# damaggu/StableKeypoints

Hardware: AMD Instinct MI355X
Metric: images/sec (token-opt step, 512², N=500 tokens) (higher is better)
Workload: dtype f32

## Files before the change

stablekeypoints_amd/csrc/skp_softmax.hip:

```cpp
#include "skp_common.h"

using namespace skp;

namespace {

template <int TPR, int EPT, bool VEC>
__global__ __launch_bounds__(TPR) void softmax_bwd_kernel(const float* __restrict__ P, float* __restrict__ G,
                                                          long long rows, int cols, float alpha) {
  __shared__ float sred[TPR / WAVE];
  const long long row = blockIdx.x;
  if (row >= rows) return;
  const float* p = P + row * cols;
  float* g = G + row * cols;
  static_assert(!VEC || EPT % 4 == 0, "float4 path needs EPT % 4 == 0");
  float pv[EPT], gv[EPT];
  float dot = 0.0f;
  if (VEC) {
#pragma unroll
    for (int q = 0; q < EPT / 4; ++q) {
      const int e = 4 * (threadIdx.x + q * TPR);
      float4 a = make_float4(0.f, 0.f, 0.f, 0.f), b = a;
      if (e < cols) {
        a = *reinterpret_cast<const float4*>(p + e);
        b = *reinterpret_cast<const float4*>(g + e);
      }
      pv[4 * q] = a.x; pv[4 * q + 1] = a.y; pv[4 * q + 2] = a.z; pv[4 * q + 3] = a.w;
      gv[4 * q] = b.x; gv[4 * q + 1] = b.y; gv[4 * q + 2] = b.z; gv[4 * q + 3] = b.w;
    }
  } else {
#pragma unroll
    for (int q = 0; q < EPT; ++q) {
      const int e = threadIdx.x + q * TPR;
      pv[q] = e < cols ? p[e] : 0.0f;
      gv[q] = e < cols ? g[e] : 0.0f;
    }
  }
#pragma unroll
  for (int q = 0; q < EPT; ++q) dot += pv[q] * gv[q];
  dot = wave_sum(dot);
  if (TPR > WAVE) {
    const int lane = threadIdx.x & (WAVE - 1), wid = threadIdx.x / WAVE;
    if (lane == 0) sred[wid] = dot;
    __syncthreads();
    float t = 0.0f;
#pragma unroll
    for (int w = 0; w < TPR / WAVE; ++w) t += sred[w];
    dot = t;
  }
  if (VEC) {
#pragma unroll
    for (int q = 0; q < EPT / 4; ++q) {
      const int e = 4 * (threadIdx.x + q * TPR);
      if (e < cols)
        *reinterpret_cast<float4*>(g + e) =
            make_float4(alpha * (pv[4 * q] * (gv[4 * q] - dot)), alpha * (pv[4 * q + 1] * (gv[4 * q + 1] - dot)),
                        alpha * (pv[4 * q + 2] * (gv[4 * q + 2] - dot)),
                        alpha * (pv[4 * q + 3] * (gv[4 * q + 3] - dot)));
    }
  } else {
#pragma unroll
    for (int q = 0; q < EPT; ++q) {
      const int e = threadIdx.x + q * TPR;
      if (e < cols) g[e] = alpha * (pv[q] * (gv[q] - dot));
    }
  }
}

template <int TPR, int EPT>
__global__ __launch_bounds__(TPR) void softmax_fwd_kernel(float* __restrict__ S, long long rows, int cols) {
  __shared__ float sred[2][TPR / WAVE];
  const long long row = blockIdx.x;
  if (row >= rows) return;
  float* p = S + row * cols;
  float v[EPT];
  float m = -INFINITY;
#pragma unroll
  for (int q = 0; q < EPT / 4; ++q) {
    const int e = 4 * (threadIdx.x + q * TPR);
    float4 a = make_float4(-INFINITY, -INFINITY, -INFINITY, -INFINITY);
    if (e < cols) a = *reinterpret_cast<const float4*>(p + e);
    v[4 * q] = a.x;
    v[4 * q + 1] = a.y;
    v[4 * q + 2] = a.z;
// ... 92 lines not shown
                                                          const float* __restrict__ V, const float* __restrict__ D,
                                                          float* out, int S, int L, float alpha) {
  constexpr int d = 4 * KS, dp = d + 1;
  __shared__ float sO[64 * dp], sV[64 * dp];
  const int b = blockIdx.z;
  const int r0 = blockIdx.y * 64, k0 = blockIdx.x * 64;
  const int t = threadIdx.x, lane = t & 63, w = t >> 6;
  {
    const float4* gO = reinterpret_cast<const float4*>(dO + ((size_t)b * S + r0) * d);
    const float4* gV = reinterpret_cast<const float4*>(V + ((size_t)b * L + k0) * d);
    for (int e = t; e < 64 * KS; e += 256) {
      const int row = e / KS, c = 4 * (e - row * KS);
      const float4 o = gO[e], v = gV[e];
      float* po = sO + row * dp + c;
      float* pv = sV + row * dp + c;
      po[0] = o.x; po[1] = o.y; po[2] = o.z; po[3] = o.w;
      pv[0] = v.x; pv[1] = v.y; pv[2] = v.z; pv[3] = v.w;
    }
  }
  __syncthreads();
  const float* va = sV + (16 * w + (lane & 15)) * dp + (lane >> 4);
  const float* ob = sO + (lane & 15) * dp + (lane >> 4);
  f32x4a acc[4];
#pragma unroll
  for (int bj = 0; bj < 4; ++bj) acc[bj] = f32x4a{0.f, 0.f, 0.f, 0.f};
#pragma unroll
  for (int ks = 0; ks < KS; ++ks) {
    const float a = va[4 * ks];
#pragma unroll
    for (int bj = 0; bj < 4; ++bj)
      acc[bj] = __builtin_amdgcn_mfma_f32_16x16x4f32(a, ob[16 * bj * dp + 4 * ks], acc[bj], 0, 0, 0);
  }
  const int key = k0 + 16 * w + 4 * (lane >> 4);
#pragma unroll
  for (int bj = 0; bj < 4; ++bj) {
    const int row = r0 + 16 * bj + (lane & 15);
    const float dr = D[(size_t)b * S + row];
    const size_t o = ((size_t)b * S + row) * L + key;
    const float4 p = *reinterpret_cast<const float4*>(P + o);
    *reinterpret_cast<float4*>(out + o) =
        make_float4(alpha * (p.x * (acc[bj][0] - dr)), alpha * (p.y * (acc[bj][1] - dr)),
                    alpha * (p.z * (acc[bj][2] - dr)), alpha * (p.w * (acc[bj][3] - dr)));
  }
}
}

extern "C" int skp_attn_dscore(const float* P, const float* dO, const float* V, const float* D, float* out, int BH,
                               int S, int L, int d, float alpha, void* stream) {
  SKP_CHECK_ARG(P && dO && V && D && out, "null pointer");
  SKP_CHECK_ARG(BH > 0 && S > 0 && L > 0 && d > 0, "non-positive shape");
  SKP_CHECK_ARG(S % 64 == 0 && L % 64 == 0, "S and L must be multiples of 64");
  SKP_CHECK_ARG(((reinterpret_cast<uintptr_t>(P) | reinterpret_cast<uintptr_t>(dO) | reinterpret_cast<uintptr_t>(V) |
                  reinterpret_cast<uintptr_t>(out)) & 15) == 0,
                "tensors must be 16-byte aligned");
  SKP_CHECK_ARG(BH <= 65535 && S / 64 <= 65535, "grid too large");
  const dim3 grid((unsigned)(L / 64), (unsigned)(S / 64), (unsigned)BH);
  hipStream_t st = as_stream(stream);
#define SKP_DS(K) hipLaunchKernelGGL((attn_dscore_kernel<K>), grid, dim3(256), 0, st, P, dO, V, D, out, S, L, alpha)
  switch (d) {
    case 40: SKP_DS(10); break;
    case 64: SKP_DS(16); break;
    case 80: SKP_DS(20); break;
    case 160: SKP_DS(40); break;
    default: SKP_CHECK_ARG(false, "head dim must be 40, 64, 80 or 160");
  }
#undef SKP_DS
  SKP_LAUNCH_CHECK();
  return SKP_OK;
}

struct AttnLay {
  long long sb;
  int rs;
  template <typename T>
  __device__ __forceinline__ T* at(T* base, int bh, int H, int d) const {
    const int b = bh / H;
    return base + (size_t)b * sb + (size_t)(bh - b * H) * d;
  }
};

namespace {

template <int KS, int DB>
__global__ __launch_bounds__(256) void attn_fwd_kernel(const float* __restrict__ Q, const float* __restrict__ K,
                                                       const float* __restrict__ V, float* __restrict__ O,
                                                       float2* __restrict__ ST, int S, int L, float scale, int H,
                                                       AttnLay lq, AttnLay lk, AttnLay lv, AttnLay lo) {
  constexpr int d = 4 * KS, dp = d + 1;
  __shared__ float sK[64 * dp], sV[64 * 16 * DB];
  const int b = blockIdx.y;
  const int r0 = blockIdx.x * 64;
  const int t = threadIdx.x, lane = t & 63, w = t >> 6;
  const int row = r0 + 16 * w + (lane & 15);
  const float* Qb = lq.at(Q, b, H, d);
  const float* Kb = lk.at(K, b, H, d);
  const float* Vb = lv.at(V, b, H, d);
  float qv[KS];
  {
    const float* q = Qb + (size_t)row * lq.rs + (lane >> 4);
#pragma unroll
    for (int ks = 0; ks < KS; ++ks) qv[ks] = q[4 * ks] * scale;
  }
  f32x4a o[DB];
#pragma unroll
  for (int db = 0; db < DB; ++db) o[db] = f32x4a{0.f, 0.f, 0.f, 0.f};
  float m = -INFINITY, l = 0.0f;
  for (int k0 = 0; k0 < L; k0 += 64) {
    __syncthreads();
    {
      for (int e = t; e < 64 * KS; e += 256) {
        const int key = e / KS, c = 4 * (e - key * KS);
        float4 kk = make_float4(0.f, 0.f, 0.f, 0.f), vv = kk;
        if (k0 + key < L) {
          kk = *reinterpret_cast<const float4*>(Kb + (size_t)(k0 + key) * lk.rs + c);
          vv = *reinterpret_cast<const float4*>(Vb + (size_t)(k0 + key) * lv.rs + c);
        }
        float* pk = sK + key * dp + c;
        pk[0] = kk.x; pk[1] = kk.y; pk[2] = kk.z; pk[3] = kk.w;
        *reinterpret_cast<float4*>(sV + key * 16 * DB + c) = vv;
      }
      if constexpr (16 * DB > d)
        for (int e = t; e < 64 * (16 * DB - d); e += 256) {
          const int key = e / (16 * DB - d), c = d + (e - key * (16 * DB - d));
          sV[key * 16 * DB + c] = 0.0f;
        }
    }
    __syncthreads();
    f32x4a s4[4];
#pragma unroll
    for (int c = 0; c < 4; ++c) {
      s4[c] = f32x4a{0.f, 0.f, 0.f, 0.f};
      const float* kr = sK + (16 * c + (lane & 15)) * dp + (lane >> 4);
#pragma unroll
      for (int ks = 0; ks < KS; ++ks) s4[c] = __builtin_amdgcn_mfma_f32_16x16x4f32(kr[4 * ks], qv[ks], s4[c], 0, 0, 0);
    }
    if (k0 + 64 > L) {
#pragma unroll
      for (int c = 0; c < 4; ++c)
#pragma unroll
        for (int r = 0; r < 4; ++r)
          if (k0 + 16 * c + 4 * (lane >> 4) + r >= L) s4[c][r] = -INFINITY;
    }
    float bm = -INFINITY;
#pragma unroll
    for (int c = 0; c < 4; ++c) bm = fmaxf(bm, fmaxf(fmaxf(s4[c][0], s4[c][1]), fmaxf(s4[c][2], s4[c][3])));
    bm = fmaxf(bm, __shfl_xor(bm, 16, 64));
    bm = fmaxf(bm, __shfl_xor(bm, 32, 64));
    const float mn = fmaxf(m, bm);
    const float corr = __expf(m - mn);
    float bs = 0.0f;
#pragma unroll
    for (int c = 0; c < 4; ++c)
#pragma unroll
      for (int r = 0; r < 4; ++r) {
        s4[c][r] = __expf(s4[c][r] - mn);
        bs += s4[c][r];
      }
    bs += __shfl_xor(bs, 16, 64);
    bs += __shfl_xor(bs, 32, 64);
    l = l * corr + bs;
    m = mn;
#pragma unroll
    for (int db = 0; db < DB; ++db) o[db] *= corr;
#pragma unroll
    for (int c = 0; c < 4; ++c)
#pragma unroll
      for (int r = 0; r < 4; ++r) {
        const float* vr = sV + (16 * c + 4 * (lane >> 4) + r) * 16 * DB + (lane & 15);
#pragma unroll
        for (int db = 0; db < DB; ++db)
          o[db] = __builtin_amdgcn_mfma_f32_16x16x4f32(vr[16 * db], s4[c][r], o[db], 0, 0, 0);
      }
  }
  const float inv = 1.0f / l;
  float* orow = lo.at(O, b, H, d) + (size_t)row * lo.rs;
#pragma unroll
  for (int db = 0; db < DB; ++db) {
    const int dd = 16 * db + 4 * (lane >> 4);
    if (dd < d) *reinterpret_cast<float4*>(orow + dd) = make_float4(o[db][0] * inv, o[db][1] * inv, o[db][2] * inv, o[db][3] * inv);
  }
  if (ST != nullptr && lane < 16) ST[(size_t)b * S + row] = make_float2(m, inv);
}

}

namespace {
int attn_fwd_launch(const float* Q, AttnLay lq, const float* K, AttnLay lk, const float* V, AttnLay lv, float* O,
                    AttnLay lo, float* stats, int BH, int H, int S, int L, int d, float scale, void* stream) {
  SKP_CHECK_ARG(Q && K && V && O, "null pointer");
  SKP_CHECK_ARG(BH > 0 && H > 0 && BH % H == 0 && S > 0 && L > 0, "non-positive shape");
  SKP_CHECK_ARG(S % 64 == 0, "S must be a multiple of 64");
  SKP_CHECK_ARG(BH <= 65535, "grid too large");
  SKP_CHECK_ARG(((reinterpret_cast<uintptr_t>(K) | reinterpret_cast<uintptr_t>(V) | reinterpret_cast<uintptr_t>(O)) &
                 15) == 0,
                "tensors must be 16-byte aligned");
  SKP_CHECK_ARG(((lk.rs | lv.rs | lo.rs | lk.sb | lv.sb | lo.sb) & 3) == 0, "K, V, O strides must be multiples of 4");
  SKP_CHECK_ARG((reinterpret_cast<uintptr_t>(stats) & 7) == 0, "stats must be 8-byte aligned");
  const dim3 grid((unsigned)(S / 64), (unsigned)BH);
  hipStream_t st = as_stream(stream);
  float2* ST = reinterpret_cast<float2*>(stats);
#define SKP_AF(KS_, DB_)                                                                                        \
  hipLaunchKernelGGL((attn_fwd_kernel<KS_, DB_>), grid, dim3(256), 0, st, Q, K, V, O, ST, S, L, scale, H, lq, lk, lv, \
                     lo)
  switch (d) {
    case 40: SKP_AF(10, 3); break;
    case 64: SKP_AF(16, 4); break;
    case 80: SKP_AF(20, 5); break;
    default: SKP_CHECK_ARG(false, "head dim must be 40, 64 or 80");
  }
#undef SKP_AF
  SKP_LAUNCH_CHECK();
  return SKP_OK;
}
AttnLay contig(int rows, int d) { return AttnLay{(long long)rows * d, d}; }
}

extern "C" int skp_attn_fwd(const float* Q, const float* K, const float* V, float* O, float* stats, int BH, int S,
                            int L, int d, float scale, void* stream) {
  return attn_fwd_launch(Q, contig(S, d), K, contig(L, d), V, contig(L, d), O, contig(S, d), stats, BH, 1, S, L, d,
                         scale, stream);
}

extern "C" int skp_attn_fwd_bshd(const float* Q, long long q_sb, int q_rs, const float* K, long long k_sb, int k_rs,
                                 const float* V, long long v_sb, int v_rs, float* O, long long o_sb, int o_rs,
                                 float* stats, int B, int H, int S, int L, int d, float scale, void* stream) {
  SKP_CHECK_ARG(B > 0 && H > 0 && (long long)B * H <= 65535, "bad B, H");
  return attn_fwd_launch(Q, AttnLay{q_sb, q_rs}, K, AttnLay{k_sb, k_rs}, V, AttnLay{v_sb, v_rs}, O, AttnLay{o_sb, o_rs},
                         stats, B * H, H, S, L, d, scale, stream);
}

namespace {

template <int KS, int DB, int WPE, bool RC>
__global__ __launch_bounds__(256) __attribute__((amdgpu_waves_per_eu(WPE, WPE))) void attn_bwd_kv_kernel(
    const float* __restrict__ P, const float* __restrict__ dO, const float* __restrict__ Q, const float* __restrict__ V,
    const float* __restrict__ D, float* __restrict__ dS, float* __restrict__ dV, float* __restrict__ dK, int S, int L,
    float alpha, const float* __restrict__ Kt, const float2* __restrict__ ST, float scale, int H, AttnLay lo, AttnLay lq,
    AttnLay lk, AttnLay lv, AttnLay ldv, AttnLay ldk) {
  constexpr int d = 4 * KS, dp = d + 1, dq = 16 * DB + 1;
  __shared__ float sV[64 * dp];
  __shared__ float sK[RC ? 64 * dp : 1];
  __shared__ float2 sST[2][RC ? 64 : 1];
  __shared__ float sO[2][64 * dq], sQ[2][64 * dq];
  __shared__ float sD[2][64];
  const int b = blockIdx.y, k0 = blockIdx.x * 64;
  const int t = threadIdx.x, lane = t & 63, w = t >> 6;
  const float* Vb = lv.at(V, b, H, d);
  const float* dOb = lo.at(dO, b, H, d);
  const float* Qb = lq.at(Q, b, H, d);
  {
    for (int e = t; e < 64 * KS; e += 256) {
      const int key = e / KS, c = 4 * (e - key * KS);
      const bool in = k0 + key < L;
      const float4 v = in ? *reinterpret_cast<const float4*>(Vb + (size_t)(k0 + key) * lv.rs + c)
                          : make_float4(0.f, 0.f, 0.f, 0.f);
      float* p = sV + key * dp + c;
      p[0] = v.x; p[1] = v.y; p[2] = v.z; p[3] = v.w;
      if constexpr (RC) {
        const float4 kk = in ? *reinterpret_cast<const float4*>(lk.at(Kt, b, H, d) + (size_t)(k0 + key) * lk.rs + c)
                             : make_float4(0.f, 0.f, 0.f, 0.f);
        float* pk = sK + key * dp + c;
        pk[0] = kk.x; pk[1] = kk.y; pk[2] = kk.z; pk[3] = kk.w;
      }
    }
    for (int e = t; e < 64 * (dq - d); e += 256) {
      const int row = e / (dq - d), c = d + (e - row * (dq - d));
      sO[0][row * dq + c] = 0.0f; sO[1][row * dq + c] = 0.0f;
      sQ[0][row * dq + c] = 0.0f; sQ[1][row * dq + c] = 0.0f;
    }
  }
  constexpr int NPF = (64 * KS + 255) / 256;
  float4 fo[NPF], fq[NPF];
  float fd = 0.0f;
  float2 fst = make_float2(0.0f, 0.0f);
  const int rl = 16 * w + 4 * (lane >> 4);
  auto fetch = [&](int r0) {
#pragma unroll
    for (int j = 0; j < NPF; ++j) {
      const int e = t + 256 * j;
      if (e < 64 * KS) {
        const int row = e / KS, c = 4 * (e - row * KS);
        fo[j] = *reinterpret_cast<const float4*>(dOb + (size_t)(r0 + row) * lo.rs + c);
        fq[j] = *reinterpret_cast<const float4*>(Qb + (size_t)(r0 + row) * lq.rs + c);
      }
    }
    if (t < 64) {
      fd = D[(size_t)b * S + r0 + t];
      if constexpr (RC) fst = ST[(size_t)b * S + r0 + t];
    }
  };
  auto stash = [&](int buf) {
#pragma unroll
    for (int j = 0; j < NPF; ++j) {
      const int e = t + 256 * j;
      if (e < 64 * KS) {
        const int row = e / KS, c = 4 * (e - row * KS);
        float* po = sO[buf] + row * dq + c;
        float* pq = sQ[buf] + row * dq + c;
        po[0] = fo[j].x; po[1] = fo[j].y; po[2] = fo[j].z; po[3] = fo[j].w;
        pq[0] = fq[j].x; pq[1] = fq[j].y; pq[2] = fq[j].z; pq[3] = fq[j].w;
      }
    }
    if (t < 64) {
      sD[buf][t] = fd;
      if constexpr (RC) sST[buf][t] = fst;
    }
  };
  const float* Pl = P + ((size_t)b * S + rl) * L + k0 + (lane & 15);
  float* dSl = dS + ((size_t)b * S + rl) * L + k0 + (lane & 15);
  f32x4a pc[4];
  if constexpr (!RC) {
#pragma unroll
    for (int bj = 0; bj < 4; ++bj)
#pragma unroll
      for (int r = 0; r < 4; ++r) pc[bj][r] = Pl[(size_t)r * L + 16 * bj];
  }
  fetch(0);
  stash(0);
  f32x4a dv[DB][4], dk[DB][4];
#pragma unroll
  for (int db = 0; db < DB; ++db)
#pragma unroll
    for (int bj = 0; bj < 4; ++bj) {
      dv[db][bj] = f32x4a{0.f, 0.f, 0.f, 0.f};
      dk[db][bj] = f32x4a{0.f, 0.f, 0.f, 0.f};
    }
  for (int r0 = 0, buf = 0; r0 < S; r0 += 64, buf ^= 1) {
    __syncthreads();
    const bool more = r0 + 64 < S;
    f32x4a pn[4];
    if (more) {
      fetch(r0 + 64);
      if constexpr (!RC) {
        const float* Pn = Pl + (size_t)(r0 + 64) * L;
#pragma unroll
        for (int bj = 0; bj < 4; ++bj)
#pragma unroll
          for (int r = 0; r < 4; ++r) pn[bj][r] = Pn[(size_t)r * L + 16 * bj];
      }
    }
    const float* tO = sO[buf];
    const float* tQ = sQ[buf];
    f32x4a dp4[4];
    {
      const float* oa = tO + (16 * w + (lane & 15)) * dq + (lane >> 4);
      const float* vb = sV + (lane & 15) * dp + (lane >> 4);
#pragma unroll
      for (int bj = 0; bj < 4; ++bj) dp4[bj] = f32x4a{0.f, 0.f, 0.f, 0.f};
#pragma unroll
      for (int ks = 0; ks < KS; ++ks) {
        const float a = oa[4 * ks];
#pragma unroll
        for (int bj = 0; bj < 4; ++bj)
          dp4[bj] = __builtin_amdgcn_mfma_f32_16x16x4f32(a, vb[16 * bj * dp + 4 * ks], dp4[bj], 0, 0, 0);
      }
    }
    if constexpr (RC) {
      f32x4a sc[4];
      const float* qa = tQ + (16 * w + (lane & 15)) * dq + (lane >> 4);
      const float* kb = sK + (lane & 15) * dp + (lane >> 4);
#pragma unroll
      for (int bj = 0; bj < 4; ++bj) sc[bj] = f32x4a{0.f, 0.f, 0.f, 0.f};
#pragma unroll
      for (int ks = 0; ks < KS; ++ks) {
        const float a = qa[4 * ks];
#pragma unroll
        for (int bj = 0; bj < 4; ++bj)
          sc[bj] = __builtin_amdgcn_mfma_f32_16x16x4f32(a, kb[16 * bj * dp + 4 * ks], sc[bj], 0, 0, 0);
      }
#pragma unroll
      for (int r = 0; r < 4; ++r) {
        const float2 st = sST[buf][rl + r];
#pragma unroll
        for (int bj = 0; bj < 4; ++bj)
          pc[bj][r] = k0 + 16 * bj + (lane & 15) < L ? __expf(sc[bj][r] * scale - st.x) * st.y : 0.0f;
      }
    }
    f32x4a s4[4];
    float* dSr = dSl + (size_t)r0 * L;
#pragma unroll
    for (int r = 0; r < 4; ++r) {
      const float Dr = sD[buf][rl + r];
#pragma unroll
      for (int bj = 0; bj < 4; ++bj) {
        const float sv = alpha * (pc[bj][r] * (dp4[bj][r] - Dr));
        if (!RC || k0 + 16 * bj + (lane & 15) < L) dSr[(size_t)r * L + 16 * bj] = sv;
        s4[bj][r] = sv;
      }
    }
#pragma unroll
    for (int r = 0; r < 4; ++r) {
      const float* orow = tO + (rl + r) * dq + (lane & 15);
      const float* qrow = tQ + (rl + r) * dq + (lane & 15);
#pragma unroll
      for (int db = 0; db < DB; ++db) {
        const float ao = orow[16 * db], aq = qrow[16 * db];
#pragma unroll
        for (int bj = 0; bj < 4; ++bj) {
          dv[db][bj] = __builtin_amdgcn_mfma_f32_16x16x4f32(ao, pc[bj][r], dv[db][bj], 0, 0, 0);
          dk[db][bj] = __builtin_amdgcn_mfma_f32_16x16x4f32(aq, s4[bj][r], dk[db][bj], 0, 0, 0);
        }
      }
    }
    if (more) {
      stash(buf ^ 1);
      if constexpr (!RC) {
#pragma unroll
        for (int bj = 0; bj < 4; ++bj) pc[bj] = pn[bj];
      }
    }
  }
  __syncthreads();
  float* red = sO[0];
  for (int m = 0; m < 2; ++m) {
#pragma unroll
    for (int db = 0; db < DB; ++db)
#pragma unroll
      for (int bj = 0; bj < 4; ++bj) {
        const f32x4a val = m == 0 ? dv[db][bj] : dk[db][bj];
        *reinterpret_cast<float4*>(red + (w * 64 + lane) * 4) = make_float4(val[0], val[1], val[2], val[3]);
        __syncthreads();
        if (w == 0) {
          float4 acc = *reinterpret_cast<const float4*>(red + lane * 4);
#pragma unroll
          for (int ww = 1; ww < 4; ++ww) {
            const float4 x = *reinterpret_cast<const float4*>(red + (ww * 64 + lane) * 4);
            acc.x += x.x; acc.y += x.y; acc.z += x.z; acc.w += x.w;
          }
          const int dd = 16 * db + 4 * (lane >> 4);
          const int key = k0 + 16 * bj + (lane & 15);
          if (dd < d && key < L) {
            float* dst = m == 0 ? ldv.at(dV, b, H, d) + (size_t)key * ldv.rs : ldk.at(dK, b, H, d) + (size_t)key * ldk.rs;
            *reinterpret_cast<float4*>(dst + dd) = acc;
          }
        }
        __syncthreads();
      }
  }
}

}

extern "C" int skp_attn_bwd_kv(const float* P, const float* dO, const float* Q, const float* V, const float* D,
                               float* dS, float* dV, float* dK, int BH, int S, int L, int d, float alpha,
                               void* stream) {
  SKP_CHECK_ARG(P && dO && Q && V && D && dS && dV && dK, "null pointer");
  SKP_CHECK_ARG(BH > 0 && S > 0 && L > 0, "non-positive shape");
  SKP_CHECK_ARG(S % 64 == 0 && L % 64 == 0, "S and L must be multiples of 64");
  SKP_CHECK_ARG(BH <= 65535, "grid too large");
  SKP_CHECK_ARG(((reinterpret_cast<uintptr_t>(dO) | reinterpret_cast<uintptr_t>(Q) | reinterpret_cast<uintptr_t>(V) |
                  reinterpret_cast<uintptr_t>(dV) | reinterpret_cast<uintptr_t>(dK)) & 15) == 0,
                "tensors must be 16-byte aligned");
  const dim3 grid((unsigned)(L / 64), (unsigned)BH);
  hipStream_t st = as_stream(stream);
  const AttnLay ls = contig(S, d), ll = contig(L, d);
  switch (d) {
#define SKP_BKV(KS_, DB_, W_) \
  hipLaunchKernelGGL((attn_bwd_kv_kernel<KS_, DB_, W_, false>), grid, dim3(256), 0, st, P, dO, Q, V, D, dS, dV, dK, S, L, \
                     alpha, nullptr, nullptr, 0.0f, 1, ls, ls, ll, ll, ll, ll)
    case 40: SKP_BKV(10, 3, 2); break;
    case 64: SKP_BKV(16, 4, 1); break;
    case 80: SKP_BKV(20, 5, 1); break;
#undef SKP_BKV
    default: SKP_CHECK_ARG(false, "head dim must be 40, 64 or 80");
  }
  SKP_LAUNCH_CHECK();
  return SKP_OK;
}

namespace {
int attn_bwd_flash_launch(const float* Q, AttnLay lq, const float* K, AttnLay lk, const float* V, AttnLay lv,
                          const float* dO, AttnLay lo, const float* stats, const float* D, float* dS, float* dV,
                          AttnLay ldv, float* dK, AttnLay ldk, int BH, int H, int S, int L, int d, float scale,
                          void* stream) {
  SKP_CHECK_ARG(Q && K && V && dO && stats && D && dS && dV && dK, "null pointer");
  SKP_CHECK_ARG(BH > 0 && H > 0 && BH % H == 0 && S > 0 && L > 0, "non-positive shape");
  SKP_CHECK_ARG(S % 64 == 0, "S must be a multiple of 64");
  SKP_CHECK_ARG(BH <= 65535, "grid too large");
  SKP_CHECK_ARG(((reinterpret_cast<uintptr_t>(dO) | reinterpret_cast<uintptr_t>(Q) | reinterpret_cast<uintptr_t>(K) |
                  reinterpret_cast<uintptr_t>(V) | reinterpret_cast<uintptr_t>(dV) | reinterpret_cast<uintptr_t>(dK)) &
                 15) == 0 && (reinterpret_cast<uintptr_t>(stats) & 7) == 0,
                "tensors must be 16-byte aligned (stats 8-byte)");
  SKP_CHECK_ARG(((lq.rs | lk.rs | lv.rs | lo.rs | ldv.rs | ldk.rs | lq.sb | lk.sb | lv.sb | lo.sb | ldv.sb | ldk.sb) & 3) == 0,
                "strides must be multiples of 4");
  const dim3 grid((unsigned)((L + 63) / 64), (unsigned)BH);
  hipStream_t st = as_stream(stream);
  const float2* ST = reinterpret_cast<const float2*>(stats);
  switch (d) {
#define SKP_BFL(KS_, DB_, W_) \
  hipLaunchKernelGGL((attn_bwd_kv_kernel<KS_, DB_, W_, true>), grid, dim3(256), 0, st, nullptr, dO, Q, V, D, dS, dV, dK, \
                     S, L, scale, K, ST, scale, H, lo, lq, lk, lv, ldv, ldk)
    case 40: SKP_BFL(10, 3, 2); break;
    case 64: SKP_BFL(16, 4, 1); break;
    case 80: SKP_BFL(20, 5, 1); break;
#undef SKP_BFL
    default: SKP_CHECK_ARG(false, "head dim must be 40, 64 or 80");
  }
  SKP_LAUNCH_CHECK();
  return SKP_OK;
}
}

extern "C" int skp_attn_bwd_flash(const float* Q, const float* K, const float* V, const float* dO, const float* stats,
                                  const float* D, float* dS, float* dV, float* dK, int BH, int S, int L, int d, float scale,
                                  void* stream) {
  const AttnLay ls = contig(S, d), ll = contig(L, d);
  return attn_bwd_flash_launch(Q, ls, K, ll, V, ll, dO, ls, stats, D, dS, dV, ll, dK, ll, BH, 1, S, L, d, scale, stream);
}

extern "C" int skp_attn_bwd_flash_bshd(const float* Q, long long q_sb, int q_rs, const float* K, long long k_sb,
                                       int k_rs, const float* V, long long v_sb, int v_rs, const float* dO,
                                       long long o_sb, int o_rs, const float* stats, const float* D, float* dS,
                                       float* dV, long long dv_sb, int dv_rs, float* dK, long long dk_sb, int dk_rs,
                                       int B, int H, int S, int L, int d, float scale, void* stream) {
  SKP_CHECK_ARG(B > 0 && H > 0 && (long long)B * H <= 65535, "bad B, H");
  return attn_bwd_flash_launch(Q, AttnLay{q_sb, q_rs}, K, AttnLay{k_sb, k_rs}, V, AttnLay{v_sb, v_rs}, dO,
                               AttnLay{o_sb, o_rs}, stats, D, dS, dV, AttnLay{dv_sb, dv_rs}, dK, AttnLay{dk_sb, dk_rs},
                               B * H, H, S, L, d, scale, stream);
}
```

stablekeypoints_amd/ops.py:

```python
import ctypes
import os

import torch

from . import _lib
from ._lib import call, ptr, stream

F32 = torch.float32

_TIMER = None


def set_kernel_timer(timer):
    global _TIMER
    _TIMER = timer


class _NoTimer:
    def __enter__(self):
        return self

    def __exit__(self, *a):
        return False

# ... 1042 lines not shown
        dy = _c(dy)
        dres = None if dpass is None else _c16(dpass)
        C = x.shape[-1]
        dx = torch.empty_like(x)
        call("skp_layernorm_bwd_add", ptr(x), ptr(dy), ptr(w), ptr(stats), x.numel() // C, C, ptr(dres), ptr(dx),
             stream(x.device))
        return dx, None, None, None


def layer_norm_res(x, weight, bias, eps):
    _lib.require_device(x)
    C = x.shape[-1]
    if (x.dtype != F32 or C % 4 or C > 2048 or weight is None or bias is None or weight.requires_grad
            or bias.requires_grad or x.numel() == 0 or x.numel() // C < LN_MIN_ROWS):
        return torch.nn.functional.layer_norm(x, (C,), weight, bias, eps), x
    return LayerNormRes.apply(x, weight, bias, float(eps))


LN_MIN_ROWS = 2048


def layer_norm(x, weight, bias, eps):
    _lib.require_device(x)
    C = x.shape[-1]
    if (x.dtype != F32 or C % 4 or C > 2048 or weight is None or bias is None or weight.requires_grad
            or bias.requires_grad or x.numel() == 0 or x.numel() // C < LN_MIN_ROWS):
        return torch.nn.functional.layer_norm(x, (C,), weight, bias, eps)
    return LayerNormFn.apply(x, weight, bias, float(eps))


class Geglu(torch.autograd.Function):

    @staticmethod
    def forward(ctx, h):
        h = _c(h)
        I = h.shape[-1] // 2
        out = torch.empty(*h.shape[:-1], I, device=h.device, dtype=F32)
        call("skp_geglu_fwd", ptr(h), h.numel() // h.shape[-1], I, ptr(out), stream(h.device))
        ctx.save_for_backward(h)
        return out

    @staticmethod
    def backward(ctx, dout):
        (h,) = ctx.saved_tensors
        dout = _c(dout)
        dh = torch.empty_like(h)
        call("skp_geglu_bwd", ptr(h), ptr(dout), h.numel() // h.shape[-1], h.shape[-1] // 2, ptr(dh),
             stream(h.device))
        return dh


def geglu(h):
    _lib.require_device(h)
    if h.dtype != F32 or h.shape[-1] % 8:
        x, gate = h.chunk(2, dim=-1)
        return x * torch.nn.functional.gelu(gate)
    return Geglu.apply(h)


ATTN_FLASH = (40, 64)


class FlashAttention(torch.autograd.Function):

    @staticmethod
    def forward(ctx, q, k, v, scale):
        BH, S, d = q.shape
        L = k.shape[1]
        out = torch.empty_like(q)
        stats = torch.empty(BH, S, 2, device=q.device, dtype=F32)
        call("skp_attn_fwd", ptr(q), ptr(k), ptr(v), ptr(out), ptr(stats), BH, S, L, d, float(scale),
             stream(q.device))
        ctx.save_for_backward(q, k, v, out, stats)
        ctx.scale = scale
        return out

    @staticmethod
    def backward(ctx, dout):
        q, k, v, out, stats = ctx.saved_tensors
        dout = dout.contiguous()
        BH, S, d = q.shape
        L = k.shape[1]
        D = (dout * out).sum(-1)
        ds = torch.empty(BH, S, L, device=q.device, dtype=F32)
        dv, dk = torch.empty_like(v), torch.empty_like(k)
        call("skp_attn_bwd_flash", ptr(q), ptr(k), ptr(v), ptr(dout), ptr(stats), ptr(D), ptr(ds), ptr(dv), ptr(dk),
             BH, S, L, d, float(ctx.scale), stream(q.device))
        dq = torch.bmm(ds, k) if ctx.needs_input_grad[0] else None
        return dq, dk if ctx.needs_input_grad[1] else None, dv if ctx.needs_input_grad[2] else None, None


def math_attention(q, k, v, scale):
    _lib.require_device(q, k, v)
    BH, S, d = q.shape
    L = k.shape[1]
    if (d in ATTN_FLASH and S % 64 == 0 and q.dtype == F32
            and all(t.dtype == F32 and t.is_contiguous() and t.data_ptr() % 16 == 0 for t in (q, k, v))):
        return FlashAttention.apply(q, k, v, float(scale))
    return MathAttention.apply(q, k, v, float(scale))


ATTN_BSHD = True


def _lay(t):
    return int(t.stride(0)), int(t.stride(1))


def _bshd_ok(q, k, v, H):
    B, S, C = q.shape
    if not ATTN_BSHD or C % H or S % 64 or k.shape[-1] != C or v.shape[-1] != C:
        return False
    return all(t.is_cuda and t.dtype == F32 and t.dim() == 3 and t.stride(2) == 1 and t.stride(1) % 4 == 0
               and t.stride(0) % 4 == 0 and t.data_ptr() % 16 == 0 for t in (q, k, v))


class FlashAttentionBSHD(torch.autograd.Function):

    @staticmethod
    def forward(ctx, q, k, v, H, scale):
        B, S, C = q.shape
        L = k.shape[1]
        d = C // H
        out = torch.empty(B, S, C, device=q.device, dtype=F32)
        stats = torch.empty(B * H, S, 2, device=q.device, dtype=F32)
        call("skp_attn_fwd_bshd", ptr(q), *_lay(q), ptr(k), *_lay(k), ptr(v), *_lay(v), ptr(out), S * C, C, ptr(stats),
             B, H, S, L, d, float(scale), stream(q.device))
        ctx.save_for_backward(q, k, v, out, stats)
        ctx.H, ctx.scale = H, scale
        return out

    @staticmethod
    def backward(ctx, dout):
        q, k, v, out, stats = ctx.saved_tensors
        H, scale = ctx.H, ctx.scale
        dout = _c16(dout)
        B, S, C = q.shape
        L = k.shape[1]
        d = C // H
        D = (dout.view(B, S, H, d) * out.view(B, S, H, d)).sum(-1).transpose(1, 2).contiguous()
        ds = torch.empty(B * H, S, L, device=q.device, dtype=F32)
        dv = torch.empty(B, L, C, device=q.device, dtype=F32)
        dk = torch.empty(B, L, C, device=q.device, dtype=F32)
        call("skp_attn_bwd_flash_bshd", ptr(q), *_lay(q), ptr(k), *_lay(k), ptr(v), *_lay(v), ptr(dout), S * C, C,
             ptr(stats), ptr(D), ptr(ds), ptr(dv), L * C, C, ptr(dk), L * C, C, B, H, S, L, d, float(scale),
             stream(q.device))
        dq = None
        if ctx.needs_input_grad[0]:
            k4 = k.view(k.shape[0], L, H, d).transpose(1, 2).expand(B, H, L, d)
            dq = torch.matmul(ds.view(B, H, S, L), k4).transpose(1, 2).reshape(B, S, C)
        return (dq, dk if ctx.needs_input_grad[1] else None, dv if ctx.needs_input_grad[2] else None, None, None)


def attention_heads(q, k, v, H, scale):
    if not _bshd_ok(q, k, v, H):
        return None
    B, S, C = q.shape
    d = C // H
    if torch.is_grad_enabled() and (q.requires_grad or k.requires_grad or v.requires_grad):
        if d not in ATTN_FLASH or k.stride(0) != 0:
            return None
        return FlashAttentionBSHD.apply(q, k, v, int(H), float(scale))
    if d not in (40, 64, 80):
        return None
    out = torch.empty(B, S, C, device=q.device, dtype=F32)
    call("skp_attn_fwd_bshd", ptr(q), *_lay(q), ptr(k), *_lay(k), ptr(v), *_lay(v), ptr(out), S * C, C, None,
         B, H, S, k.shape[1], d, float(scale), stream(q.device))
    return out


_QKV_W = {}


def _qkv_weight(*ws):
    key = tuple(id(w) for w in ws)
    sig = tuple((w._version, w.data_ptr()) for w in ws)
    ent = _QKV_W.get(key)
    if ent is not None and ent[0] == sig and all(r() is w for r, w in zip(ent[1], ws)):
        return ent[2]
    w3 = torch.cat([w.detach() for w in ws], 0).contiguous()
    drop = lambda _r, key=key: _QKV_W.pop(key, None)
    _QKV_W[key] = (sig, tuple(_weakref.ref(w, drop) for w in ws), w3)
    return w3


class QKVProjection(torch.autograd.Function):

    @staticmethod
    def forward(ctx, x, w3, C):
        out = torch.matmul(x, w3.t())
        ctx.save_for_backward(w3)
        ctx.C = C
        ctx.x_shape = x.shape
        ctx.set_materialize_grads(False)
        return tuple(out[..., i * C:(i + 1) * C] for i in range(w3.shape[0] // C))

    @staticmethod
    def backward(ctx, *grads):
        (w3,) = ctx.saved_tensors
        C = ctx.C
        dx = None
        for i, g in enumerate(grads):
            if g is None:
                continue
            g2 = g.reshape(-1, C)
            wi = w3[i * C:(i + 1) * C]
            if dx is None:
                dx = torch.mm(g2, wi)
            else:
                dx.addmm_(g2, wi)
        if dx is None:
            return None, None, None
        return dx.view(ctx.x_shape), None, None


QKV_FUSED = True


def qkv_projection(x, *ws):
    _lib.require_device(x)
    return QKVProjection.apply(x, _qkv_weight(*ws), int(ws[0].shape[0]))


class TokensProjIn(torch.autograd.Function):

    @staticmethod
    def forward(ctx, x, w, bias):
        B, C, HW = x.shape
        h = torch.bmm(x.transpose(1, 2), w.t().expand(B, C, w.shape[0]))
        if bias is not None:
            h.add_(bias)
# ... 552 lines not shown
```

Baseline: 45.30.

## Restage attention K/V shared layouts for vector LDS reads and skip unused dS writes

The attention forward kernel now prefetches K/V tiles into registers, writes them into a grouped/transposed LDS layout that allows float4 reads for the MFMA operands, and splits the loop into full blocks plus a masked tail. The backward kv kernel uses the same grouped layout for V/K, precomputes fetch offsets, and gains a template flag that skips writing the dense dS matrix when dq is not needed. The Python side passes a null dS in that case. This aims to cut LDS bank traffic, per-iteration index arithmetic and global writes, at the cost of higher register pressure and a new waves_per_eu hint.

```diff
diff --git a/stablekeypoints_amd/csrc/skp_softmax.hip b/stablekeypoints_amd/csrc/skp_softmax.hip
--- a/stablekeypoints_amd/csrc/skp_softmax.hip
+++ b/stablekeypoints_amd/csrc/skp_softmax.hip
@@ -1,4 +1,6 @@
 #include "skp_common.h"
+
+#include <type_traits>
 
 using namespace skp;
 
@@ -257,64 +259,119 @@
 namespace {
 
 template <int KS, int DB>
-__global__ __launch_bounds__(256) void attn_fwd_kernel(const float* __restrict__ Q, const float* __restrict__ K,
-                                                       const float* __restrict__ V, float* __restrict__ O,
-                                                       float2* __restrict__ ST, int S, int L, float scale, int H,
-                                                       AttnLay lq, AttnLay lk, AttnLay lv, AttnLay lo) {
-  constexpr int d = 4 * KS, dp = d + 1;
-  __shared__ float sK[64 * dp], sV[64 * 16 * DB];
+__global__ __launch_bounds__(256) __attribute__((amdgpu_waves_per_eu(2))) void attn_fwd_kernel(
+    const float* __restrict__ Q, const float* __restrict__ K, const float* __restrict__ V, float* __restrict__ O,
+    float2* __restrict__ ST, int S, int L, float scale, int H, AttnLay lq, AttnLay lk, AttnLay lv, AttnLay lo) {
+  constexpr int d = 4 * KS, NC = 16 * DB, KH = KS / 2, KQ = (KS + 3) / 4;
+  constexpr int GK = KS == 10 ? 12 : 20, RSK = KS == 10 ? 56 : 88;
+  static_assert(KS % 2 == 0 && GK % 4 == 0 && GK >= 4 * KQ && 3 * GK + 4 * KQ <= RSK && RSK % 4 == 0, "sK layout");
+  constexpr int NPK = (64 * KH + 255) / 256, NPV = (16 * KS + 255) / 256;
+  __shared__ __attribute__((aligned(16))) float sK[64 * RSK];
+  __shared__ __attribute__((aligned(16))) float sV[64 * NC];
   const int b = blockIdx.y;
   const int r0 = blockIdx.x * 64;
   const int t = threadIdx.x, lane = t & 63, w = t >> 6;
-  const int row = r0 + 16 * w + (lane & 15);
+  const int li = lane & 15, lg = lane >> 4;
+  const int row = r0 + 16 * w + li;
   const float* Qb = lq.at(Q, b, H, d);
-  const float* Kb = lk.at(K, b, H, d);
-  const float* Vb = lv.at(V, b, H, d);
+  const float* Kp = lk.at(K, b, H, d);
+  const float* Vp = lv.at(V, b, H, d);
   float qv[KS];
   {
-    const float* q = Qb + (size_t)row * lq.rs + (lane >> 4);
+    const float* q = Qb + (size_t)row * lq.rs + lg;
 #pragma unroll
     for (int ks = 0; ks < KS; ++ks) qv[ks] = q[4 * ks] * scale;
+  }
+  int gk[NPK], sk[NPK], gv[NPV], sv[NPV];
+#pragma unroll
+  for (int j = 0; j < NPK; ++j) {
+    const int e = t + 256 * j, key = e / KH, p = e - key * KH;
+    gk[j] = key * lk.rs + 8 * p;
+    sk[j] = key * RSK + 2 * p;
+  }
+#pragma unroll
+  for (int j = 0; j < NPV; ++j) {
+    const int e = 255 - t + 256 * j, kq = e / KS, cq = e - kq * KS;
+    gv[j] = 4 * kq * lv.rs + 4 * cq;
+    sv[j] = (kq * NC + 4 * cq) * 4;
+  }
+  auto has_k = [&](int j) { return 256 * (j + 1) <= 64 * KH || t + 256 * j < 64 * KH; };
+  auto has_v = [&](int j) { return 256 * (j + 1) <= 16 * KS || 255 - t + 256 * j < 16 * KS; };
+  if constexpr (NC > d) {
+    constexpr int PQ = NC - d;
+    for (int e = t; e < 16 * PQ; e += 256) {
+      const int kq = e / PQ, c = d + (e - kq * PQ);
+      *reinterpret_cast<float4*>(sV + (kq * NC + c) * 4) = make_float4(0.f, 0.f, 0.f, 0.f);
+    }
   }
   f32x4a o[DB];
 #pragma unroll
   for (int db = 0; db < DB; ++db) o[db] = f32x4a{0.f, 0.f, 0.f, 0.f};
   float m = -INFINITY, l = 0.0f;
-  for (int k0 = 0; k0 < L; k0 += 64) {
+  auto block = [&](const int rem, auto rg) {
+    constexpr bool RG = decltype(rg)::value;
+    float4 rk[NPK][2], rv[NPV][4];
+    const float4 zero = make_float4(0.f, 0.f, 0.f, 0.f);
+#pragma unroll
+    for (int j = 0; j < NPK; ++j)
+      if (has_k(j)) {
+        bool in = true;
+        if constexpr (RG) in = (t + 256 * j) / KH < rem;
+        rk[j][0] = zero; rk[j][1] = zero;
+        if (in) {
+          rk[j][0] = *reinterpret_cast<const float4*>(Kp + gk[j]);
+          rk[j][1] = *reinterpret_cast<const float4*>(Kp + gk[j] + 4);
+        }
+      }
+#pragma unroll
+    for (int j = 0; j < NPV; ++j)
+      if (has_v(j)) {
+#pragma unroll
+        for (int x = 0; x < 4; ++x) {
+          bool in = true;
+          if constexpr (RG) in = 4 * ((255 - t + 256 * j) / KS) + x < rem;
+          rv[j][x] = zero;
+          if (in) rv[j][x] = *reinterpret_cast<const float4*>(Vp + (size_t)x * lv.rs + gv[j]);
+        }
+      }
     __syncthreads();
-    {
-      for (int e = t; e < 64 * KS; e += 256) {
-        const int key = e / KS, c = 4 * (e - key * KS);
-        float4 kk = make_float4(0.f, 0.f, 0.f, 0.f), vv = kk;
-        if (k0 + key < L) {
-          kk = *reinterpret_cast<const float4*>(Kb + (size_t)(k0 + key) * lk.rs + c);
-          vv = *reinterpret_cast<const float4*>(Vb + (size_t)(k0 + key) * lv.rs + c);
-        }
-        float* pk = sK + key * dp + c;
-        pk[0] = kk.x; pk[1] = kk.y; pk[2] = kk.z; pk[3] = kk.w;
-        *reinterpret_cast<float4*>(sV + key * 16 * DB + c) = vv;
-      }
-      if constexpr (16 * DB > d)
-        for (int e = t; e < 64 * (16 * DB - d); e += 256) {
-          const int key = e / (16 * DB - d), c = d + (e - key * (16 * DB - d));
-          sV[key * 16 * DB + c] = 0.0f;
-        }
-    }
+#pragma unroll
+    for (int j = 0; j < NPK; ++j)
+      if (has_k(j)) {
+        float* pk = sK + sk[j];
+        *reinterpret_cast<float2*>(pk) = make_float2(rk[j][0].x, rk[j][1].x);
+        *reinterpret_cast<float2*>(pk + GK) = make_float2(rk[j][0].y, rk[j][1].y);
+        *reinterpret_cast<float2*>(pk + 2 * GK) = make_float2(rk[j][0].z, rk[j][1].z);
+        *reinterpret_cast<float2*>(pk + 3 * GK) = make_float2(rk[j][0].w, rk[j][1].w);
+      }
+#pragma unroll
+    for (int j = 0; j < NPV; ++j)
+      if (has_v(j)) {
+        float4* pv = reinterpret_cast<float4*>(sV + sv[j]);
+        pv[0] = make_float4(rv[j][0].x, rv[j][1].x, rv[j][2].x, rv[j][3].x);
+        pv[1] = make_float4(rv[j][0].y, rv[j][1].y, rv[j][2].y, rv[j][3].y);
+        pv[2] = make_float4(rv[j][0].z, rv[j][1].z, rv[j][2].z, rv[j][3].z);
+        pv[3] = make_float4(rv[j][0].w, rv[j][1].w, rv[j][2].w, rv[j][3].w);
+      }
     __syncthreads();
     f32x4a s4[4];
 #pragma unroll
     for (int c = 0; c < 4; ++c) {
       s4[c] = f32x4a{0.f, 0.f, 0.f, 0.f};
-      const float* kr = sK + (16 * c + (lane & 15)) * dp + (lane >> 4);
-#pragma unroll
-      for (int ks = 0; ks < KS; ++ks) s4[c] = __builtin_amdgcn_mfma_f32_16x16x4f32(kr[4 * ks], qv[ks], s4[c], 0, 0, 0);
-    }
-    if (k0 + 64 > L) {
+      const f32x4a* kr = reinterpret_cast<const f32x4a*>(sK + (16 * c + li) * RSK + lg * GK);
+      f32x4a kk[KQ];
+#pragma unroll
+      for (int q = 0; q < KQ; ++q) kk[q] = kr[q];
+#pragma unroll
+      for (int ks = 0; ks < KS; ++ks)
+        s4[c] = __builtin_amdgcn_mfma_f32_16x16x4f32(kk[ks >> 2][ks & 3], qv[ks], s4[c], 0, 0, 0);
+    }
+    if constexpr (RG) {
 #pragma unroll
       for (int c = 0; c < 4; ++c)
 #pragma unroll
         for (int r = 0; r < 4; ++r)
-          if (k0 + 16 * c + 4 * (lane >> 4) + r >= L) s4[c][r] = -INFINITY;
+          if (16 * c + 4 * lg + r >= rem) s4[c][r] = -INFINITY;
     }
     float bm = -INFINITY;
 #pragma unroll
@@ -338,20 +395,28 @@
 #pragma unroll
     for (int db = 0; db < DB; ++db) o[db] *= corr;
 #pragma unroll
-    for (int c = 0; c < 4; ++c)
-#pragma unroll
-      for (int r = 0; r < 4; ++r) {
-        const float* vr = sV + (16 * c + 4 * (lane >> 4) + r) * 16 * DB + (lane & 15);
+    for (int c = 0; c < 4; ++c) {
+      const f32x4a* vr = reinterpret_cast<const f32x4a*>(sV + ((4 * c + lg) * NC + li) * 4);
+      f32x4a vv[DB];
+#pragma unroll
+      for (int db = 0; db < DB; ++db) vv[db] = vr[16 * db];
+#pragma unroll
+      for (int r = 0; r < 4; ++r)
 #pragma unroll
         for (int db = 0; db < DB; ++db)
-          o[db] = __builtin_amdgcn_mfma_f32_16x16x4f32(vr[16 * db], s4[c][r], o[db], 0, 0, 0);
-      }
-  }
+          o[db] = __builtin_amdgcn_mfma_f32_16x16x4f32(vv[db][r], s4[c][r], o[db], 0, 0, 0);
+    }
+    Kp += (size_t)64 * lk.rs;
+    Vp += (size_t)64 * lv.rs;
+  };
+  int k0 = 0;
+  for (; k0 + 64 <= L; k0 += 64) block(64, std::false_type{});
+  if (k0 < L) block(L - k0, std::true_type{});
   const float inv = 1.0f / l;
   float* orow = lo.at(O, b, H, d) + (size_t)row * lo.rs;
 #pragma unroll
   for (int db = 0; db < DB; ++db) {
-    const int dd = 16 * db + 4 * (lane >> 4);
+    const int dd = 16 * db + 4 * lg;
     if (dd < d) *reinterpret_cast<float4*>(orow + dd) = make_float4(o[db][0] * inv, o[db][1] * inv, o[db][2] * inv, o[db][3] * inv);
   }
   if (ST != nullptr && lane < 16) ST[(size_t)b * S + row] = make_float2(m, inv);
@@ -370,6 +435,7 @@
                  15) == 0,
                 "tensors must be 16-byte aligned");
   SKP_CHECK_ARG(((lk.rs | lv.rs | lo.rs | lk.sb | lv.sb | lo.sb) & 3) == 0, "K, V, O strides must be multiples of 4");
+  SKP_CHECK_ARG(lk.rs > 0 && lv.rs > 0 && lk.rs < (1 << 24) && lv.rs < (1 << 24), "K, V row strides must be in (0, 2^24)");
   SKP_CHECK_ARG((reinterpret_cast<uintptr_t>(stats) & 7) == 0, "stats must be 8-byte aligned");
   const dim3 grid((unsigned)(S / 64), (unsigned)BH);
   hipStream_t st = as_stream(stream);
@@ -406,15 +472,17 @@
 
 namespace {
 
-template <int KS, int DB, int WPE, bool RC>
+template <int KS, int DB, int WPE, bool RC, bool WDS = true>
 __global__ __launch_bounds__(256) __attribute__((amdgpu_waves_per_eu(WPE, WPE))) void attn_bwd_kv_kernel(
     const float* __restrict__ P, const float* __restrict__ dO, const float* __restrict__ Q, const float* __restrict__ V,
     const float* __restrict__ D, float* __restrict__ dS, float* __restrict__ dV, float* __restrict__ dK, int S, int L,
     float alpha, const float* __restrict__ Kt, const float2* __restrict__ ST, float scale, int H, AttnLay lo, AttnLay lq,
     AttnLay lk, AttnLay lv, AttnLay ldv, AttnLay ldk) {
-  constexpr int d = 4 * KS, dp = d + 1, dq = 16 * DB + 1;
-  __shared__ float sV[64 * dp];
-  __shared__ float sK[RC ? 64 * dp : 1];
+  constexpr int d = 4 * KS, dq = 16 * DB + 1, KH = KS / 2, KQ = (KS + 3) / 4;
+  constexpr int GK = KS == 10 ? 12 : 20, RSK = KS == 10 ? 56 : 88;
+  static_assert(KS % 2 == 0 && GK % 4 == 0 && GK >= 4 * KQ && 3 * GK + 4 * KQ <= RSK && RSK % 4 == 0, "sV / sK layout");
+  __shared__ __attribute__((aligned(16))) float sV[64 * RSK];
+  __shared__ __attribute__((aligned(16))) float sK[RC ? 64 * RSK : 4];
   __shared__ float2 sST[2][RC ? 64 : 1];
   __shared__ float sO[2][64 * dq], sQ[2][64 * dq];
   __shared__ float sD[2][64];
@@ -424,19 +492,22 @@
   const float* dOb = lo.at(dO, b, H, d);
   const float* Qb = lq.at(Q, b, H, d);
   {
-    for (int e = t; e < 64 * KS; e += 256) {
-      const int key = e / KS, c = 4 * (e - key * KS);
+    auto stage = [&](const float* src, float* dst, bool in) {
+      float4 x = make_float4(0.f, 0.f, 0.f, 0.f), y = x;
+      if (in) {
+        x = *reinterpret_cast<const float4*>(src);
+        y = *reinterpret_cast<const float4*>(src + 4);
+      }
+      *reinterpret_cast<float2*>(dst) = make_float2(x.x, y.x);
+      *reinterpret_cast<float2*>(dst + GK) = make_float2(x.y, y.y);
+      *reinterpret_cast<float2*>(dst + 2 * GK) = make_float2(x.z, y.z);
+      *reinterpret_cast<float2*>(dst + 3 * GK) = make_float2(x.w, y.w);
+    };
+    for (int e = t; e < 64 * KH; e += 256) {
+      const int key = e / KH, p = e - key * KH;
       const bool in = k0 + key < L;
-      const float4 v = in ? *reinterpret_cast<const float4*>(Vb + (size_t)(k0 + key) * lv.rs + c)
-                          : make_float4(0.f, 0.f, 0.f, 0.f);
-      float* p = sV + key * dp + c;
-      p[0] = v.x; p[1] = v.y; p[2] = v.z; p[3] = v.w;
-      if constexpr (RC) {
-        const float4 kk = in ? *reinterpret_cast<const float4*>(lk.at(Kt, b, H, d) + (size_t)(k0 + key) * lk.rs + c)
-                             : make_float4(0.f, 0.f, 0.f, 0.f);
-        float* pk = sK + key * dp + c;
-        pk[0] = kk.x; pk[1] = kk.y; pk[2] = kk.z; pk[3] = kk.w;
-      }
+      stage(Vb + (size_t)(k0 + key) * lv.rs + 8 * p, sV + key * RSK + 2 * p, in);
+      if constexpr (RC) stage(lk.at(Kt, b, H, d) + (size_t)(k0 + key) * lk.rs + 8 * p, sK + key * RSK + 2 * p, in);
     }
     for (int e = t; e < 64 * (dq - d); e += 256) {
       const int row = e / (dq - d), c = d + (e - row * (dq - d));
@@ -449,14 +520,22 @@
   float fd = 0.0f;
   float2 fst = make_float2(0.0f, 0.0f);
   const int rl = 16 * w + 4 * (lane >> 4);
+  int go[NPF], gq[NPF], so[NPF];
+#pragma unroll
+  for (int j = 0; j < NPF; ++j) {
+    const int e = t + 256 * j, row = e / KS, c = 4 * (e - row * KS);
+    go[j] = row * lo.rs + c;
+    gq[j] = row * lq.rs + c;
+    so[j] = row * dq + c;
+  }
   auto fetch = [&](int r0) {
+    const float* dOr = dOb + (size_t)r0 * lo.rs;
+    const float* Qr = Qb + (size_t)r0 * lq.rs;
 #pragma unroll
     for (int j = 0; j < NPF; ++j) {
-      const int e = t + 256 * j;
-      if (e < 64 * KS) {
-        const int row = e / KS, c = 4 * (e - row * KS);
-        fo[j] = *reinterpret_cast<const float4*>(dOb + (size_t)(r0 + row) * lo.rs + c);
-        fq[j] = *reinterpret_cast<const float4*>(Qb + (size_t)(r0 + row) * lq.rs + c);
+      if (256 * (j + 1) <= 64 * KS || t + 256 * j < 64 * KS) {
+        fo[j] = *reinterpret_cast<const float4*>(dOr + go[j]);
+        fq[j] = *reinterpret_cast<const float4*>(Qr + gq[j]);
       }
     }
     if (t < 64) {
@@ -467,11 +546,9 @@
   auto stash = [&](int buf) {
 #pragma unroll
     for (int j = 0; j < NPF; ++j) {
-      const int e = t + 256 * j;
-      if (e < 64 * KS) {
-        const int row = e / KS, c = 4 * (e - row * KS);
-        float* po = sO[buf] + row * dq + c;
-        float* pq = sQ[buf] + row * dq + c;
+      if (256 * (j + 1) <= 64 * KS || t + 256 * j < 64 * KS) {
+        float* po = sO[buf] + so[j];
+        float* pq = sQ[buf] + so[j];
         po[0] = fo[j].x; po[1] = fo[j].y; po[2] = fo[j].z; po[3] = fo[j].w;
         pq[0] = fq[j].x; pq[1] = fq[j].y; pq[2] = fq[j].z; pq[3] = fq[j].w;
       }
@@ -519,29 +596,37 @@
     f32x4a dp4[4];
     {
       const float* oa = tO + (16 * w + (lane & 15)) * dq + (lane >> 4);
-      const float* vb = sV + (lane & 15) * dp + (lane >> 4);
-#pragma unroll
-      for (int bj = 0; bj < 4; ++bj) dp4[bj] = f32x4a{0.f, 0.f, 0.f, 0.f};
-#pragma unroll
-      for (int ks = 0; ks < KS; ++ks) {
-        const float a = oa[4 * ks];
-#pragma unroll
-        for (int bj = 0; bj < 4; ++bj)
-          dp4[bj] = __builtin_amdgcn_mfma_f32_16x16x4f32(a, vb[16 * bj * dp + 4 * ks], dp4[bj], 0, 0, 0);
+      const f32x4a* vb = reinterpret_cast<const f32x4a*>(sV + (lane & 15) * RSK + (lane >> 4) * GK);
+      float a[KS];
+#pragma unroll
+      for (int ks = 0; ks < KS; ++ks) a[ks] = oa[4 * ks];
+#pragma unroll
+      for (int bj = 0; bj < 4; ++bj) {
+        dp4[bj] = f32x4a{0.f, 0.f, 0.f, 0.f};
+        f32x4a bb[KQ];
+#pragma unroll
+        for (int q = 0; q < KQ; ++q) bb[q] = vb[4 * bj * RSK + q];
+#pragma unroll
+        for (int ks = 0; ks < KS; ++ks)
+          dp4[bj] = __builtin_amdgcn_mfma_f32_16x16x4f32(a[ks], bb[ks >> 2][ks & 3], dp4[bj], 0, 0, 0);
       }
     }
     if constexpr (RC) {
       f32x4a sc[4];
       const float* qa = tQ + (16 * w + (lane & 15)) * dq + (lane >> 4);
-      const float* kb = sK + (lane & 15) * dp + (lane >> 4);
-#pragma unroll
-      for (int bj = 0; bj < 4; ++bj) sc[bj] = f32x4a{0.f, 0.f, 0.f, 0.f};
-#pragma unroll
-      for (int ks = 0; ks < KS; ++ks) {
-        const float a = qa[4 * ks];
-#pragma unroll
-        for (int bj = 0; bj < 4; ++bj)
-          sc[bj] = __builtin_amdgcn_mfma_f32_16x16x4f32(a, kb[16 * bj * dp + 4 * ks], sc[bj], 0, 0, 0);
+      const f32x4a* kb = reinterpret_cast<const f32x4a*>(sK + (lane & 15) * RSK + (lane >> 4) * GK);
+      float a[KS];
+#pragma unroll
+      for (int ks = 0; ks < KS; ++ks) a[ks] = qa[4 * ks];
+#pragma unroll
+      for (int bj = 0; bj < 4; ++bj) {
+        sc[bj] = f32x4a{0.f, 0.f, 0.f, 0.f};
+        f32x4a bb[KQ];
+#pragma unroll
+        for (int q = 0; q < KQ; ++q) bb[q] = kb[4 * bj * RSK + q];
+#pragma unroll
+        for (int ks = 0; ks < KS; ++ks)
+          sc[bj] = __builtin_amdgcn_mfma_f32_16x16x4f32(a[ks], bb[ks >> 2][ks & 3], sc[bj], 0, 0, 0);
       }
 #pragma unroll
       for (int r = 0; r < 4; ++r) {
@@ -557,10 +642,20 @@
     for (int r = 0; r < 4; ++r) {
       const float Dr = sD[buf][rl + r];
 #pragma unroll
-      for (int bj = 0; bj < 4; ++bj) {
-        const float sv = alpha * (pc[bj][r] * (dp4[bj][r] - Dr));
-        if (!RC || k0 + 16 * bj + (lane & 15) < L) dSr[(size_t)r * L + 16 * bj] = sv;
-        s4[bj][r] = sv;
+      for (int bj = 0; bj < 4; ++bj) s4[bj][r] = alpha * (pc[bj][r] * (dp4[bj][r] - Dr));
+    }
+    if constexpr (WDS) {
+      if (!RC || k0 + 64 <= L) {
+#pragma unroll
+        for (int r = 0; r < 4; ++r)
+#pragma unroll
+          for (int bj = 0; bj < 4; ++bj) dSr[(size_t)r * L + 16 * bj] = s4[bj][r];
+      } else {
+#pragma unroll
+        for (int r = 0; r < 4; ++r)
+#pragma unroll
+          for (int bj = 0; bj < 4; ++bj)
+            if (k0 + 16 * bj + (lane & 15) < L) dSr[(size_t)r * L + 16 * bj] = s4[bj][r];
       }
     }
 #pragma unroll
@@ -648,7 +743,7 @@
                           const float* dO, AttnLay lo, const float* stats, const float* D, float* dS, float* dV,
                           AttnLay ldv, float* dK, AttnLay ldk, int BH, int H, int S, int L, int d, float scale,
                           void* stream) {
-  SKP_CHECK_ARG(Q && K && V && dO && stats && D && dS && dV && dK, "null pointer");
+  SKP_CHECK_ARG(Q && K && V && dO && stats && D && dV && dK, "null pointer");
   SKP_CHECK_ARG(BH > 0 && H > 0 && BH % H == 0 && S > 0 && L > 0, "non-positive shape");
   SKP_CHECK_ARG(S % 64 == 0, "S must be a multiple of 64");
   SKP_CHECK_ARG(BH <= 65535, "grid too large");
@@ -658,16 +753,21 @@
                 "tensors must be 16-byte aligned (stats 8-byte)");
   SKP_CHECK_ARG(((lq.rs | lk.rs | lv.rs | lo.rs | ldv.rs | ldk.rs | lq.sb | lk.sb | lv.sb | lo.sb | ldv.sb | ldk.sb) & 3) == 0,
                 "strides must be multiples of 4");
+  SKP_CHECK_ARG(lq.rs > 0 && lo.rs > 0 && lq.rs < (1 << 24) && lo.rs < (1 << 24), "Q, dO row strides must be in (0, 2^24)");
   const dim3 grid((unsigned)((L + 63) / 64), (unsigned)BH);
   hipStream_t st = as_stream(stream);
   const float2* ST = reinterpret_cast<const float2*>(stats);
   switch (d) {
-#define SKP_BFL(KS_, DB_, W_) \
-  hipLaunchKernelGGL((attn_bwd_kv_kernel<KS_, DB_, W_, true>), grid, dim3(256), 0, st, nullptr, dO, Q, V, D, dS, dV, dK, \
-                     S, L, scale, K, ST, scale, H, lo, lq, lk, lv, ldv, ldk)
+#define SKP_BFL_(KS_, DB_, W_, WDS_)                                                                                  \
+  hipLaunchKernelGGL((attn_bwd_kv_kernel<KS_, DB_, W_, true, WDS_>), grid, dim3(256), 0, st, nullptr, dO, Q, V, D, dS, dV, \
+                     dK, S, L, scale, K, ST, scale, H, lo, lq, lk, lv, ldv, ldk)
+#define SKP_BFL(KS_, DB_, W_)                \
+  if (dS != nullptr) SKP_BFL_(KS_, DB_, W_, true); \
+  else SKP_BFL_(KS_, DB_, W_, false)
     case 40: SKP_BFL(10, 3, 2); break;
     case 64: SKP_BFL(16, 4, 1); break;
     case 80: SKP_BFL(20, 5, 1); break;
+#undef SKP_BFL_
 #undef SKP_BFL
     default: SKP_CHECK_ARG(false, "head dim must be 40, 64 or 80");
   }
diff --git a/stablekeypoints_amd/ops.py b/stablekeypoints_amd/ops.py
--- a/stablekeypoints_amd/ops.py
+++ b/stablekeypoints_amd/ops.py
@@ -1148,11 +1148,11 @@
         BH, S, d = q.shape
         L = k.shape[1]
         D = (dout * out).sum(-1)
-        ds = torch.empty(BH, S, L, device=q.device, dtype=F32)
+        ds = torch.empty(BH, S, L, device=q.device, dtype=F32) if ctx.needs_input_grad[0] else None
         dv, dk = torch.empty_like(v), torch.empty_like(k)
         call("skp_attn_bwd_flash", ptr(q), ptr(k), ptr(v), ptr(dout), ptr(stats), ptr(D), ptr(ds), ptr(dv), ptr(dk),
              BH, S, L, d, float(ctx.scale), stream(q.device))
-        dq = torch.bmm(ds, k) if ctx.needs_input_grad[0] else None
+        dq = torch.bmm(ds, k) if ds is not None else None
         return dq, dk if ctx.needs_input_grad[1] else None, dv if ctx.needs_input_grad[2] else None, None
 
 
@@ -1205,14 +1205,14 @@
         L = k.shape[1]
         d = C // H
         D = (dout.view(B, S, H, d) * out.view(B, S, H, d)).sum(-1).transpose(1, 2).contiguous()
-        ds = torch.empty(B * H, S, L, device=q.device, dtype=F32)
+        ds = torch.empty(B * H, S, L, device=q.device, dtype=F32) if ctx.needs_input_grad[0] else None
         dv = torch.empty(B, L, C, device=q.device, dtype=F32)
         dk = torch.empty(B, L, C, device=q.device, dtype=F32)
         call("skp_attn_bwd_flash_bshd", ptr(q), *_lay(q), ptr(k), *_lay(k), ptr(v), *_lay(v), ptr(dout), S * C, C,
              ptr(stats), ptr(D), ptr(ds), ptr(dv), L * C, C, ptr(dk), L * C, C, B, H, S, L, d, float(scale),
              stream(q.device))
         dq = None
-        if ctx.needs_input_grad[0]:
+        if ds is not None:
             k4 = k.view(k.shape[0], L, H, d).transpose(1, 2).expand(B, H, L, d)
             dq = torch.matmul(ds.view(B, H, S, L), k4).transpose(1, 2).reshape(B, S, C)
         return (dq, dk if ctx.needs_input_grad[1] else None, dv if ctx.needs_input_grad[2] else None, None, None)
```

Result: no change. 45.72 (median of 6 runs) (+0.9%).
